# AaltoPML/PPBO

Measured on NVIDIA B200. Metric: ppbo_iteration_ms, lower is better.
Workload: dtype f64

## Files before the change

ppbo_b200/csrc/acq.cu:

```cuda
#include <algorithm>
#include <cmath>
#include <cstdlib>
#include <vector>

#include "../../include/ppbo_b200.h"
#include "common.cuh"
#include "gemm_f64.cuh"
#include "linalg.cuh"
#include "philox.cuh"

namespace ppbo {

extern int g_tuning[16];
int kernel_matvec(int kind, const double* X1, int n1, const double* X2, int n2, int D, const double* ls_h, double sigma_f,
                  const double* alpha, double* mu, double* partial, cudaStream_t st);
int kernel_matrix_raw(int kind, const double* X1, int n1, const double* X2, int n2, int D, const double* ls_h,
                      double sigma_f, double scale, double diag_add, double* out, long long ld, cudaStream_t st);

__global__ void __launch_bounds__(256) pred_diff_kernel(const double* __restrict__ Kc, long long ldk, int PT, int Q, int m,
                                                        const double* __restrict__ arrow, double* __restrict__ Ut,
                                                        long long ldu) {
    const int u = blockIdx.x * blockDim.x + threadIdx.x, p = blockIdx.y;
    if (u >= Q * m) return;
    const int q = u / m, j = u % m;
// ... 153 lines not shown
#pragma unroll
            for (int d = 0; d < RM_MAX_D; ++d)
                if (d < D) gl[d] = fma(c, w[d], gl[d]);
        }
        for (int o = 16; o > 0; o >>= 1) val += __shfl_xor_sync(0xffffffffu, val, o);
        if (lane == 0) red[warp][RM_MAX_D] = val;
#pragma unroll
        for (int d = 0; d < RM_MAX_D; ++d) {
            if (d < D) {
                double v = gl[d];
                for (int o = 16; o > 0; o >>= 1) v += __shfl_xor_sync(0xffffffffu, v, o);
                if (lane == 0) red[warp][d] = v;
            }
        }
        __syncthreads();
        if (tid <= D) {
            const int k = (tid == D) ? RM_MAX_D : tid;
            const double v = amp * ((red[0][k] + red[1][k]) + (red[2][k] + red[3][k]));
            if (tid == D) fval_s = v;
            else gv[tid] = v;
        }
        __syncthreads();
    };
    if (tid < D) x[tid] = fmin(fmax(x0[tid], 0.0), 1.0);
    __syncthreads();
    eval(x, g);
    double f = fval_s;
    double gmax = 0.0;
    for (int d = 0; d < D; ++d) gmax = fmax(gmax, fabs(g[d]));
    double t = 0.05 / fmax(gmax, 1e-12);
    int it = 0;
    for (; it < max_iter; ++it) {
        double pg = 0.0;
        for (int d = 0; d < D; ++d) pg = fmax(pg, fabs(fmin(fmax(x[d] + g[d], 0.0), 1.0) - x[d]));
        if (pg <= gtol) break;
        double ft = f, slope = 0.0;
        int tries = 0;
        for (;; ++tries) {
            __syncthreads();
            if (tid < D) xt[tid] = fmin(fmax(x[tid] + t * g[tid], 0.0), 1.0);
            __syncthreads();
            slope = 0.0;
            for (int d = 0; d < D; ++d) slope = fma(g[d], xt[d] - x[d], slope);
            eval(xt, gt);
            ft = fval_s;
            if (ft >= f + 1e-4 * slope || tries >= 30) break;
            t *= 0.5;
        }
        if (!(ft >= f)) break;
        double ss = 0.0, sy = 0.0;
        for (int d = 0; d < D; ++d) {
            const double sd = xt[d] - x[d], yd = gt[d] - g[d];
            ss = fma(sd, sd, ss);
            sy = fma(sd, yd, sy);
        }
        __syncthreads();
        if (tid < D) { x[tid] = xt[tid]; g[tid] = gt[tid]; }
        __syncthreads();
        f = ft;
        t = (sy < 0.0) ? fmin(fmax(-ss / sy, 1e-8), 1e4) : 2.0 * t;
        if (ss == 0.0) break;
    }
    if (tid < D) xout[(long long)blockIdx.x * D + tid] = x[tid];
    if (tid == 0) {
        fout[blockIdx.x] = f;
        if (iters_out) iters_out[blockIdx.x] = it;
    }
}
__global__ void rff_maximize_select_kernel(const double* __restrict__ xall, const double* __restrict__ fall, int S, int R, int D,
                                           double* __restrict__ xbest, double* __restrict__ fbest) {
    const int s = blockIdx.x * blockDim.x + threadIdx.x;
    if (s >= S) return;
    int br = 0;
    double bf = fall[(long long)s * R];
    for (int r = 1; r < R; ++r) {
        const double v = fall[(long long)s * R + r];
        if (v > bf) { bf = v; br = r; }
    }
    fbest[s] = bf;
    for (int d = 0; d < D; ++d) xbest[(long long)s * D + d] = xall[((long long)s * R + br) * D + d];
}

constexpr int FV_SLICES = 8, FV_COLS = 128;
__global__ void __launch_bounds__(256) rff_fvals_partial_kernel(const double* __restrict__ Phi, long long ld, int F, int N,
                                                                const double* __restrict__ omega, double* __restrict__ part,
                                                                const double* __restrict__ skip) {
    __shared__ double red[FV_COLS];
    if (skip && *skip != 0.0) return;
    const int c = threadIdx.x & (FV_COLS - 1), half = threadIdx.x >> 7;
    const int i = blockIdx.x * FV_COLS + c;
    const int per = (F + FV_SLICES - 1) / FV_SLICES;
    const int f0 = blockIdx.y * per, f1 = min(F, f0 + per);
    double s0 = 0.0, s1 = 0.0;
    if (i < N) {
        int f = f0 + half;
        for (; f + 2 < f1; f += 4) {
            s0 = fma(Phi[(long long)f * ld + i], omega[f], s0);
            s1 = fma(Phi[(long long)(f + 2) * ld + i], omega[f + 2], s1);
        }
        for (; f < f1; f += 2) s0 = fma(Phi[(long long)f * ld + i], omega[f], s0);
    }
    if (half == 1) red[c] = s0 + s1;
    __syncthreads();
    if (half == 0 && i < N) part[(long long)blockIdx.y * N + i] = (s0 + s1) + red[c];
}
__global__ void __launch_bounds__(256) rff_fvals_combine_kernel(const double* __restrict__ part, int N, double* __restrict__ y) {
    const int i = blockIdx.x * blockDim.x + threadIdx.x;
    if (i >= N) return;
    double s = 0.0;
#pragma unroll
    for (int k = 0; k < FV_SLICES; ++k) s += part[(long long)k * N + i];
    y[i] = s;
}
static int launch_rff_fvals(const double* Phi, long long ld, int F, int N, const double* omega, double* part, double* y,
                            cudaStream_t st, const double* skip = nullptr) {
    PPBO_CL rff_fvals_partial_kernel<<<dim3(ceil_div(N, FV_COLS), FV_SLICES), 256, 0, st>>>(Phi, ld, F, N, omega, part, skip);
    PPBO_CL rff_fvals_combine_kernel<<<ceil_div(N, 256), 256, 0, st>>>(part, N, y);
    PPBO_LAUNCH_CHECK();
    return PPBO_OK;
}
__global__ void __launch_bounds__(256) rff_grad_hess_kernel(const double* __restrict__ Phi, long long ld, int F, int Q, int m,
                                                            const double* __restrict__ omega, const double* __restrict__ beta,
                                                            const double* __restrict__ arrow, double* __restrict__ grad,
                                                            double* __restrict__ hdiag, const double* __restrict__ skip) {
    if (skip && *skip != 0.0) return;
    const int f = (blockIdx.x * blockDim.x + threadIdx.x) >> 5, lane = threadIdx.x & 31;
    if (f >= F) return;
    const double* ph = Phi + (long long)f * ld;
    const int N = Q * (m + 1), M = Q * m;
    double g = 0.0, h = 0.0;
    if (grad) for (int i = lane; i < N; i += 32) g = fma(beta[i], ph[i], g);
    if (hdiag)
        for (int u = lane; u < M; u += 32) {
            const int q = u / m, j = u % m;
            const double d = ph[(long long)q * (m + 1) + 1 + j] - ph[(long long)q * (m + 1)];
            h = fma(arrow[u], d * d, h);
        }
    for (int o = 16; o > 0; o >>= 1) {
        g += __shfl_xor_sync(0xffffffffu, g, o);
        h += __shfl_xor_sync(0xffffffffu, h, o);
    }
    if (lane == 0) {
        if (grad) grad[f] = -omega[f] + g;
        if (hdiag) hdiag[f] = -1.0 - h;
    }
}
__global__ void __launch_bounds__(256) rff_grad_kernel(const double* __restrict__ Phi, long long ld, int F, int N,
                                                       const double* __restrict__ omega, const double* __restrict__ beta,
                                                       double* __restrict__ grad, const double* __restrict__ skip) {
    __shared__ double part[8];
    if (skip && *skip != 0.0) return;
    const int warp = threadIdx.x >> 5, lane = threadIdx.x & 31;
    const int f = blockIdx.x * 2 + (warp >> 2), qtr = warp & 3;
    double g0 = 0.0, g1 = 0.0;
    if (f < F) {
        const double* ph = Phi + (long long)f * ld;
        const int per = ((N + 3) / 4 + 31) / 32 * 32, i0 = qtr * per, i1 = min(N, i0 + per);
        int i = i0 + lane;
        for (; i + 32 < i1; i += 64) {
            g0 = fma(beta[i], ph[i], g0);
            g1 = fma(beta[i + 32], ph[i + 32], g1);
        }
        if (i < i1) g0 = fma(beta[i], ph[i], g0);
    }
    double g = g0 + g1;
    for (int o = 16; o > 0; o >>= 1) g += __shfl_xor_sync(0xffffffffu, g, o);
    if (lane == 0) part[warp] = g;
    __syncthreads();
    if (threadIdx.x < 2) {
        const int ff = blockIdx.x * 2 + threadIdx.x;
        if (ff < F) grad[ff] = -omega[ff] + ((part[4 * threadIdx.x] + part[4 * threadIdx.x + 1]) + (part[4 * threadIdx.x + 2] + part[4 * threadIdx.x + 3]));
    }
}
__global__ void __launch_bounds__(256) rff_psi_kernel(const double* __restrict__ Phi, long long ld, int Q, int m,
                                                      const double* __restrict__ arrow, double* __restrict__ PsiT, long long ldp) {
    const int u = blockIdx.x * blockDim.x + threadIdx.x, f = blockIdx.y;
    if (u >= Q * m) return;
    const int q = u / m, j = u % m;
    const double* ph = Phi + (long long)f * ld;
    const double a = arrow[u];
    PsiT[(long long)f * ldp + u] = a > 0.0 ? sqrt(a) * (ph[(long long)q * (m + 1) + 1 + j] - ph[(long long)q * (m + 1)]) : 0.0;
}
__global__ void add_identity_kernel(double* __restrict__ A, long long ld, int n) {
    const int i = blockIdx.x * blockDim.x + threadIdx.x;
    if (i < n) A[(long long)i * ld + i] += 1.0;
}
__global__ void __launch_bounds__(1024) rff_scalars_kernel(const double* __restrict__ omega, const double* __restrict__ x, int F,
                                                           double* __restrict__ scal) {
    __shared__ double red[33];
    __shared__ double mx[2][32];
    double s = 0, m0 = 0, m1 = 0;
    for (int i = threadIdx.x; i < F; i += 1024) {
        s = fma(omega[i], omega[i], s);
        if (x) m0 = fmax(m0, fabs(x[i]));
        m1 = fmax(m1, fabs(omega[i]));
    }
    s = block_sum(s, red);
    for (int o = 16; o > 0; o >>= 1) {
        m0 = fmax(m0, __shfl_xor_sync(0xffffffffu, m0, o));
        m1 = fmax(m1, __shfl_xor_sync(0xffffffffu, m1, o));
    }
    if ((threadIdx.x & 31) == 0) { mx[0][threadIdx.x >> 5] = m0; mx[1][threadIdx.x >> 5] = m1; }
    __syncthreads();
    if (threadIdx.x == 0) {
        for (int w = 1; w < 32; ++w) { m0 = fmax(m0, mx[0][w]); m1 = fmax(m1, mx[1][w]); }
        scal[0] = -0.5 * s; scal[1] = m0; scal[2] = m1;
    }
}
__global__ void axpy_kernel(double* __restrict__ y, const double* __restrict__ x, double a, int n) {
    const int i = blockIdx.x * blockDim.x + threadIdx.x;
    if (i < n) y[i] += a * x[i];
}
__global__ void axpy_out_kernel(double* __restrict__ out, const double* __restrict__ y, const double* __restrict__ x, double a, int n) {
    const int i = blockIdx.x * blockDim.x + threadIdx.x;
    if (i < n) out[i] = y[i] + a * x[i];
}

int launch_lik_terms(const double* f, int Q, int m, double sigma, double* set_lik, double* beta, double* arrow, double* sa,
                     double* bvec, cudaStream_t st);
int launch_sum(const double* x, int n, double* out, cudaStream_t st);
int launch_linesearch_lik(const double* f, const double* df, int Q, int m, double sigma, double* part, cudaStream_t st);
constexpr int LS_STEPS = 8;

__global__ void __launch_bounds__(1024) rff_ls_scalars_kernel(const double* __restrict__ omega, const double* __restrict__ step,
                                                              int F, const double* __restrict__ part, int Q,
                                                              double* __restrict__ scal) {
    __shared__ double red_multi[32 * (3 + LS_STEPS)];
    __shared__ double mx[2][32];
    double m0 = 0, m1 = 0;
    double sums[3 + LS_STEPS];
#pragma unroll
    for (int c = 0; c < 3 + LS_STEPS; ++c) sums[c] = 0.0;
    for (int i = threadIdx.x; i < F; i += 1024) {
        const double o = omega[i], d = step[i];
        sums[0] = fma(o, o, sums[0]);
        sums[1] = fma(o, d, sums[1]);
        sums[2] = fma(d, d, sums[2]);
        m0 = fmax(m0, fabs(d));
        m1 = fmax(m1, fabs(o));
    }
    for (int q = threadIdx.x; q < Q; q += 1024) {
#pragma unroll
        for (int c = 0; c < LS_STEPS; ++c) sums[3 + c] += part[(long long)c * Q + q];
    }
    block_sum_multi<3 + LS_STEPS>(sums, red_multi);
    for (int o = 16; o > 0; o >>= 1) {
        m0 = fmax(m0, __shfl_xor_sync(0xffffffffu, m0, o));
        m1 = fmax(m1, __shfl_xor_sync(0xffffffffu, m1, o));
    }
    if ((threadIdx.x & 31) == 0) { mx[0][threadIdx.x >> 5] = m0; mx[1][threadIdx.x >> 5] = m1; }
    __syncthreads();
    if (threadIdx.x == 0) {
        for (int w = 1; w < 32; ++w) { m0 = fmax(m0, mx[0][w]); m1 = fmax(m1, mx[1][w]); }
        scal[0] = sums[0]; scal[1] = sums[1]; scal[2] = sums[2]; scal[3] = m0; scal[4] = m1;
        for (int c = 0; c < LS_STEPS; ++c) scal[8 + c] = sums[3 + c];
    }
}

__global__ void __launch_bounds__(256) rff_chord_decide_kernel(double* __restrict__ omega, const double* __restrict__ step, int F,
                                                               const double* __restrict__ scal, int m, double* __restrict__ state,
                                                               double* __restrict__ hist, int anderson) {
    __shared__ int accept_s;
    if (state[4] != 0.0) return;
    if (threadIdx.x == 0) {
        const double oo = scal[0], od = scal[1], dd = scal[2], max_step = scal[3], max_om = fmax(scal[4], 1e-300);
        const double S_cur = -0.5 * oo - scal[24] / m;
        const double S1 = -0.5 * (oo + 2.0 * od + dd) - scal[8] / m;
        const int accept = S1 >= S_cur - 1e-13 * fabs(S_cur);
        accept_s = accept;
        state[7] = accept ? 1.0 : 0.0;
        if (!accept) {
            state[4] = 3.0;
        } else {
            const double rel = max_step / max_om, prev = state[1], rel3 = state[3];
            const int n = (int)state[5];
            state[0] = S1;
            state[3] = state[2];
            state[2] = prev;
            state[1] = rel;
            state[5] = n + 1;
            hist[2 * n] = rel;
            hist[2 * n + 1] = S1;
            if (rel <= state[6]) state[4] = 1.0;
            else if (anderson) { if (rel3 < 1e300 && !(rel <= 0.2 * rel3)) state[4] = 2.0; }
            else if (!(rel <= 0.5 * prev)) state[4] = 2.0;
        }
    }
    __syncthreads();
    if (!accept_s) return;
    for (int i = threadIdx.x; i < F; i += blockDim.x) omega[i] += step[i];
}

constexpr int RAA_M = 5;
__global__ void __launch_bounds__(1024) rff_anderson_kernel(double* __restrict__ omega, const double* __restrict__ step, int F,
                                                            const double* __restrict__ state, double* __restrict__ aa,
                                                            double* __restrict__ Hh) {
    __shared__ double gam[RAA_M];
    __shared__ int nh_s;
    if (state[4] != 0.0) return;
    double* dR = Hh;
    double* dG = Hh + (long long)RAA_M * F;
    double* pr = Hh + 2LL * RAA_M * F;
    double* pg = pr + F;
    const bool plain = state[7] == 1.0;
    const double rel = state[1];
    int nh = (int)aa[0], slot = (int)aa[1];
    const double rel_prev = aa[2];
    bool have_prev = aa[3] == 1.0;
    __syncthreads();
    if (!plain || (have_prev && rel > 1.5 * rel_prev)) {
        if (threadIdx.x == 0) { aa[0] = 0.0; aa[1] = 0.0; aa[2] = rel; aa[3] = 0.0; }
        if (!plain) return;
        nh = 0;
        slot = 0;
        have_prev = false;
    }
    if (have_prev) {
        for (int i = threadIdx.x; i < F; i += 1024) {
            dR[(long long)slot * F + i] = step[i] - pr[i];
            dG[(long long)slot * F + i] = omega[i] - pg[i];
        }
        nh = min(nh + 1, RAA_M);
        slot = (slot + 1) % RAA_M;
    }
    for (int i = threadIdx.x; i < F; i += 1024) {
        pr[i] = step[i];
        pg[i] = omega[i];
    }
    __syncthreads();
    constexpr int NPAIR = RAA_M * (RAA_M + 1) / 2;
    __shared__ double red_multi[32 * (NPAIR + RAA_M)];
    double acc[NPAIR + RAA_M];
#pragma unroll
    for (int i = 0; i < NPAIR + RAA_M; ++i) acc[i] = 0.0;
    for (int k = threadIdx.x; k < F; k += 1024) {
        double dv[RAA_M];
#pragma unroll
        for (int i = 0; i < RAA_M; ++i) dv[i] = (i < nh) ? dR[(long long)i * F + k] : 0.0;
        const double rk = step[k];
        int idx = 0;
#pragma unroll
        for (int i = 0; i < RAA_M; ++i) {
#pragma unroll
            for (int j = 0; j <= i; ++j) { acc[idx] = fma(dv[i], dv[j], acc[idx]); ++idx; }
            acc[NPAIR + i] = fma(dv[i], rk, acc[NPAIR + i]);
        }
    }
    block_sum_multi<NPAIR + RAA_M>(acc, red_multi);
    double A[RAA_M][RAA_M], bb[RAA_M];
    {
        int idx = 0;
#pragma unroll
        for (int i = 0; i < RAA_M; ++i) {
#pragma unroll
            for (int j = 0; j <= i; ++j) { A[i][j] = A[j][i] = acc[idx]; ++idx; }
            bb[i] = acc[NPAIR + i];
        }
    }
    if (threadIdx.x == 0) {
        double tr = 0.0;
        for (int i = 0; i < nh; ++i) tr += A[i][i];
        for (int i = 0; i < nh; ++i) A[i][i] += 1e-10 * tr + 1e-300;
        bool ok = true;
        for (int c = 0; c < nh && ok; ++c) {
            int pv = c;
            for (int r2 = c + 1; r2 < nh; ++r2) if (fabs(A[r2][c]) > fabs(A[pv][c])) pv = r2;
            if (A[pv][c] == 0.0) { ok = false; break; }
            for (int k = 0; k < nh; ++k) { const double t = A[c][k]; A[c][k] = A[pv][k]; A[pv][k] = t; }
            { const double t = bb[c]; bb[c] = bb[pv]; bb[pv] = t; }
            for (int r2 = c + 1; r2 < nh; ++r2) {
                const double l = A[r2][c] / A[c][c];
                for (int k = c; k < nh; ++k) A[r2][k] -= l * A[c][k];
                bb[r2] -= l * bb[c];
            }
        }
        for (int i = nh - 1; i >= 0 && ok; --i) {
            double v = bb[i];
            for (int k = i + 1; k < nh; ++k) v -= A[i][k] * gam[k];
            gam[i] = v / A[i][i];
            if (!(fabs(gam[i]) < 1e3)) ok = false;
        }
        nh_s = ok ? nh : 0;
        aa[0] = ok ? nh : 0;
        aa[1] = ok ? slot : 0;
        aa[2] = rel;
        aa[3] = 1.0;
    }
    __syncthreads();
    const int nm = nh_s;
    if (nm == 0) return;
    for (int i = threadIdx.x; i < F; i += 1024) {
        double c = 0.0;
        for (int j = 0; j < nm; ++j) c = fma(gam[j], dG[(long long)j * F + i], c);
        omega[i] -= c;
    }
}

}

using namespace ppbo;

extern "C" long long ppbo_factor_doubles(int n) { return (long long)n * n + potrf_dinv_doubles(n) ; }

extern "C" int ppbo_neg_count(const double* arrow, int M, int* idx_h, int idx_capacity, void* stream) {
    std::vector<double> a((size_t)M);
    if (readback().add(a.data(), arrow, sizeof(double) * M, (cudaStream_t)stream) != cudaSuccess ||
        readback().finish((cudaStream_t)stream) != cudaSuccess) {
        set_error("ppbo_neg_count: copy failed");
        return PPBO_ERR_CUDA;
    }
    int r = 0;
    for (int u = 0; u < M; ++u)
        if (a[u] < 0.0) {
            if (idx_h && r < idx_capacity) idx_h[r] = u;
            ++r;
        }
    return r;
}
extern "C" long long ppbo_neg_corr_doubles(int M, int r) {
    return (long long)((r + 1) / 2) + (long long)r * M + ppbo_factor_doubles(r) + 2;
}
extern "C" int ppbo_neg_corr_build(const double* G, long long ldg, int M, const double* arrow, const double* Lfac, int cap,
                                   const int* idx_h, int r, double* neg_corr, void* stream) {
    if (r <= 0) return PPBO_OK;
    PPBO_REQUIRE(cap >= M && ldg >= M, "capacity / leading dimension below M");
    cudaStream_t st = (cudaStream_t)stream;
    int* idx = reinterpret_cast<int*>(neg_corr);
    double* Ht = neg_corr + (r + 1) / 2;
    double* R = Ht + (long long)r * M;
    double* Rdinv = R + (long long)r * r;
    int* info_d = reinterpret_cast<int*>(neg_corr + ppbo_neg_corr_doubles(M, r) - 1);
    PPBO_CUDA_CHECK(cudaMemcpyAsync(idx, idx_h, sizeof(int) * r, cudaMemcpyHostToDevice, st));
    PPBO_CL neg_rows_kernel<<<dim3(ceil_div(M, 256), r), 256, 0, st>>>(G, ldg, M, arrow, idx, r, Ht, R, r);
    PPBO_LAUNCH_CHECK();
    int rc = trsm_right_lower_t(Lfac, cap, M, Lfac + (long long)cap * cap, Ht, M, r, st);
    if (rc) return rc;
    GemmOperands g{Ht, M, 0, Ht, M, 0, r, r, M};
    StoreEpilogue ep{R, r, 0, 1.0, 1.0, 0, 0, 0};
    if ((rc = launch_gemm_nt(g, ep, 1, st))) return rc;
    if ((rc = potrf_lower(R, r, r, Rdinv, info_d, st))) return rc;
    int info = 0;
    PPBO_CUDA_CHECK(readback().add(&info, info_d, sizeof(int), st));
    PPBO_CUDA_CHECK(readback().finish(st));
    if (info) { set_error("posterior precision is not positive definite (negative-coefficient block, pivot %d)", info); return info; }
    return PPBO_OK;
}

extern "C" long long ppbo_predict_workspace_bytes(int N, int Q, int m, int P, int batch) {
    const long long PT = (long long)P * batch, M = (long long)Q * m;
    return (PT * N + PT * M + PT * M + 64) * 8;
}

extern "C" long long ppbo_predict_mean_workspace_bytes(int kind, int N, int P, int batch) {
    const long long PT = (long long)P * batch;
    if (kind == PPBO_KERNEL_SE || kind == PPBO_KERNEL_RQ) return (PT * ((N + 63) / 64) + 64) * 8;
    return (PT * N + 64) * 8;
}

extern "C" int ppbo_predict(int kind, const double* X, int N, int D, const double* lengthscales_h, double sigma_f,
                            double shrinkage, int Q, int m, const double* alpha, const double* arrow, const double* Lfac, int cap,
                            const double* neg_corr, int n_neg, const double* Xp, int P, int batch, double* mu,
                            double* Sigma_p, void* workspace, long long workspace_bytes, void* stream) {
    PPBO_REQUIRE(N == Q * (m + 1), "N must equal Q (m+1)");
    PPBO_REQUIRE(Sigma_p == nullptr || cap >= Q * m, "factor capacity below Q m");
    PPBO_REQUIRE(P >= 1 && batch >= 1, "empty grid");
    PPBO_REQUIRE(workspace_bytes >= (Sigma_p ? ppbo_predict_workspace_bytes(N, Q, m, P, batch)
                                             : ppbo_predict_mean_workspace_bytes(g_tuning[11] ? PPBO_KERNEL_CAMPHOR : kind, N, P, batch)),
                 "workspace too small");
    cudaStream_t st = (cudaStream_t)stream;
    const int PT = P * batch, M = Q * m;
    double* Kc = (double*)workspace;
    double* Ut = Kc + (long long)PT * N;
    double* Ud = Ut + (long long)PT * M;
    int rc;
    if (!Sigma_p) {
        if (!mu) return PPBO_OK;
        rc = kernel_matvec(kind, Xp, PT, X, N, D, lengthscales_h, sigma_f, alpha, mu, Kc, st);
        if (rc < 0) return rc;
// ... 32 lines not shown
        StoreEpilogue e2{Sigma_p, P, (long long)P * P, 1.0, 1.0, 0, 0, 0};
        if ((rc = launch_gemm_nt(g2, e2, batch, st))) return rc;
    }
    return PPBO_OK;
}

extern "C" int ppbo_mvn_rowmax(const double* Z, long long ldz, long long strideZ, const double* Fac, long long ldf,
                               long long strideF, const double* mu, long long strideMu, int S, int P, int K, int batch,
                               double* fmax, int* arg, void* stream) {
    PPBO_REQUIRE(S >= 0 && P >= 1 && K >= 1 && batch >= 1, "shape");
    GemmOperands g{Z, ldz, strideZ, Fac, ldf, strideF, S, P, K};
    RowMaxEpilogue ep{mu, strideMu, fmax, arg, nullptr, 0, 0};
    return launch_gemm_nt_rowmax(g, ep, batch, (cudaStream_t)stream);
}

extern "C" int ppbo_acq_reduce(const double* fmax, int S, int batch, double mustar, double* out, void* stream) {
    PPBO_REQUIRE(S >= 1 && batch >= 1, "shape");
    PPBO_CL acq_reduce_kernel<<<batch, 1024, 0, (cudaStream_t)stream>>>(fmax, S, mustar, nullptr, out);
    PPBO_LAUNCH_CHECK();
    return PPBO_OK;
}

extern "C" int ppbo_acq_reduce_dev(const double* fmax, int S, int batch, const double* mustar_dev, double* out, void* stream) {
    PPBO_REQUIRE(S >= 1 && batch >= 1 && mustar_dev != nullptr, "shape");
    PPBO_CL acq_reduce_kernel<<<batch, 1024, 0, (cudaStream_t)stream>>>(fmax, S, 0.0, mustar_dev, out);
    PPBO_LAUNCH_CHECK();
    return PPBO_OK;
}

extern "C" int ppbo_vec_max(const double* x, long long n, int accumulate, double* out, void* stream) {
    PPBO_REQUIRE(n >= 0 && out != nullptr, "shape");
    PPBO_CL vec_max_kernel<<<1, 1024, 0, (cudaStream_t)stream>>>(x, n, accumulate, out);
    PPBO_LAUNCH_CHECK();
    return PPBO_OK;
}

extern "C" int ppbo_rff_features(const double* W, const double* b, int F, int D, const double* X, int n, double sigma_f,
                                 double* Phi, long long ld, int feature_major, void* stream) {
    PPBO_REQUIRE(F >= 1 && D >= 1 && n >= 0, "shape");
    if (n == 0) return PPBO_OK;
    const double amp = sqrt(2.0 * sigma_f * sigma_f / F);
    dim3 grid = feature_major ? dim3(ceil_div(n, 256), F) : dim3(ceil_div(F, 256), n);
    PPBO_REQUIRE(grid.y <= 65535, "too many rows for one launch");
    PPBO_CL rff_features_kernel<<<grid, 256, sizeof(double) * D, (cudaStream_t)stream>>>(W, b, F, D, X, n, amp, Phi, ld, feature_major);
    PPBO_LAUNCH_CHECK();
    return PPBO_OK;
}

extern "C" int ppbo_rff_jacobian(const double* W, const double* b, int F, int D, const double* x, double sigma_f, double* J,
                                 void* stream) {
    const double amp = sqrt(2.0 * sigma_f * sigma_f / F);
    PPBO_CL rff_jacobian_kernel<<<ceil_div(F, 128), 128, 0, (cudaStream_t)stream>>>(W, b, F, D, x, amp, J);
    PPBO_LAUNCH_CHECK();
    return PPBO_OK;
}

extern "C" int ppbo_rff_value_grad(const double* W, const double* b, int F, int D, const double* omega, const double* x,
                                   double sigma_f, double* out, void* stream) {
    PPBO_REQUIRE(F >= 1 && D >= 1 && D <= PPBO_MAX_D, "shape");
    const double amp = sqrt(2.0 * sigma_f * sigma_f / F);
    PPBO_CL rff_value_grad_kernel<<<1, 256, 0, (cudaStream_t)stream>>>(W, b, F, D, omega, x, amp, out);
    PPBO_LAUNCH_CHECK();
    return PPBO_OK;
}

extern "C" int ppbo_rff_maximize(const double* W, const double* b, int F, int D, double sigma_f, const double* Omega, long long ldo,
                                 int S, const double* X0, int R, int max_iter, double gtol, double* xbest, double* fbest,
                                 double* work, void* stream) {
    PPBO_REQUIRE(F >= 1 && D >= 1 && D <= RM_MAX_D, "D must be in [1, 32]");
    PPBO_REQUIRE(S >= 0 && R >= 1 && max_iter >= 0 && gtol >= 0 && work != nullptr, "arguments");
    if (S == 0) return PPBO_OK;
    cudaStream_t st = (cudaStream_t)stream;
    const double amp = sqrt(2.0 * sigma_f * sigma_f / F);
    double* xall = work;
    double* fall = work + (long long)S * R * D;
    PPBO_CL rff_maximize_kernel<<<S * R, RM_THREADS, 0, st>>>(W, b, F, D, amp, Omega, ldo, X0, R, max_iter, gtol, xall, fall, nullptr);
    PPBO_CL rff_maximize_select_kernel<<<ceil_div(S, 128), 128, 0, st>>>(xall, fall, S, R, D, xbest, fbest);
    PPBO_LAUNCH_CHECK();
    return PPBO_OK;
}

extern "C" long long ppbo_rff_workspace_bytes(int F, int Q, int m) {
    const long long N = (long long)Q * (m + 1), M = (long long)Q * m;
    return ((3 + FV_SLICES) * N + 2 * M + Q * 9 + 64 + (long long)F * M + ppbo_factor_doubles(F) + 4 * (long long)F + 2 * CHOL_NB +
            blockinv_doubles(F) + (2LL * RAA_M + 2) * F + 8) * 8;
}

struct RffWs {
    double *fvals, *dfv, *fpart, *beta, *arrow, *setlik, *scal, *PsiT, *H, *grad, *step, *trial, *tmp, *binv, *aaH, *aa;
    void carve(double* p, int F, int Q, int m) {
        const long long N = (long long)Q * (m + 1), M = (long long)Q * m;
        fvals = p; p += N;
        dfv = p; p += N;
        fpart = p; p += (long long)FV_SLICES * N;
        beta = p; p += N;
        arrow = p; p += 2 * M;
        setlik = p; p += 9LL * Q;
        scal = p; p += 64;
        PsiT = p; p += (long long)F * M;
        H = p; p += ppbo_factor_doubles(F);
        grad = p; p += F;
        step = p; p += F + CHOL_NB;
        trial = p; p += F;
        tmp = p; p += F;
        aaH = p; p += (2LL * RAA_M + 2) * F;
        aa = p; p += 8;
        binv = p;
    }
};

static int rff_eval(const double* Phi, long long ld, int F, int Q, int m, double sigma, const double* omega, RffWs& ws,
                    double* grad, double* hdiag, bool want_arrow, double* lik_sum_dev, cudaStream_t st, const double* skip = nullptr) {
    const int N = Q * (m + 1);
    launch_rff_fvals(Phi, ld, F, N, omega, ws.fpart, ws.fvals, st, skip);
    launch_lik_terms(ws.fvals, Q, m, sigma, ws.setlik, ws.beta, want_arrow ? ws.arrow : nullptr, nullptr, nullptr, st);
    launch_sum(ws.setlik, Q, lik_sum_dev, st);
    if (grad && !hdiag)
        PPBO_CL rff_grad_kernel<<<ceil_div(F, 2), 256, 0, st>>>(Phi, ld, F, N, omega, ws.beta, grad, skip);
    else if (grad || hdiag)
        PPBO_CL rff_grad_hess_kernel<<<ceil_div(F, 8), 256, 0, st>>>(Phi, ld, F, Q, m, omega, ws.beta, ws.arrow, grad, hdiag, skip);
    PPBO_LAUNCH_CHECK();
    return PPBO_OK;
}

extern "C" int ppbo_rff_objective(const double* Phi_X, long long ld, int F, int Q, int m, double sigma, const double* omega,
                                  double* S_out, double* grad, double* hess_diag, void* workspace, long long workspace_bytes,
                                  void* stream) {
    PPBO_REQUIRE(workspace_bytes >= ppbo_rff_workspace_bytes(F, Q, m), "workspace too small");
    cudaStream_t st = (cudaStream_t)stream;
    RffWs ws;
    ws.carve((double*)workspace, F, Q, m);
    int rc = rff_eval(Phi_X, ld, F, Q, m, sigma, omega, ws, grad, hess_diag, true, ws.scal + 8, st);
    if (rc) return rc;
    if (S_out) {
        PPBO_CL rff_scalars_kernel<<<1, 1024, 0, st>>>(omega, nullptr, F, ws.scal);
        double h[9];
        PPBO_CUDA_CHECK(readback().add(h, ws.scal, sizeof(h), st));
        PPBO_CUDA_CHECK(readback().finish(st));
        *S_out = h[0] - h[8] / m;
    }
    return PPBO_OK;
}

extern "C" long long ppbo_rff_factor_cache_doubles(int F) { return ppbo_factor_doubles(F) + blockinv_doubles(F); }

extern "C" int ppbo_rff_fit(const double* Phi_X, long long ld, int F, int Q, int m, double sigma, const double* omega0,
                            int max_iter, double tol, double* factor_cache, int warm_factor, double* omega_map, double* hess_diag,
                            void* workspace, long long workspace_bytes, double* stats_h, void* stream) {
    PPBO_REQUIRE(workspace_bytes >= ppbo_rff_workspace_bytes(F, Q, m), "workspace too small");
    PPBO_REQUIRE(!warm_factor || (factor_cache != nullptr && omega0 != nullptr), "a warm factor needs the cache and omega0");
    cudaStream_t st = (cudaStream_t)stream;
    const int M = Q * m;
    RffWs ws;
    ws.carve((double*)workspace, F, Q, m);
    if (factor_cache) {
        ws.H = factor_cache;
        ws.binv = factor_cache + ppbo_factor_doubles(F);
    }
    double* Hdinv = ws.H + (long long)F * F;
    int* info_d = reinterpret_cast<int*>(ws.scal + 32);
    PPBO_CUDA_CHECK(cudaMemsetAsync(info_d, 0, sizeof(int), st));
    if (omega0) PPBO_CUDA_CHECK(cudaMemcpyAsync(omega_map, omega0, sizeof(double) * F, cudaMemcpyDeviceToDevice, st));
    else PPBO_CUDA_CHECK(cudaMemsetAsync(omega_map, 0, sizeof(double) * F, st));
    int rc, it = 0, info = 0, n_factor = 0, n_chord = 0;
    double h[32], S_cur = NAN, last_rel = INFINITY;
    const int N = Q * (m + 1);
    double* part = ws.setlik + Q;
    const double CHORD_REL = 0.25;
    const bool trace = getenv("PPBO_TRACE") != nullptr;
    bool refactor = !warm_factor, binv_valid = warm_factor == 2;
    constexpr int RFF_BATCH_MAX = 8;
    double* state_d = ws.scal + 40;
    double* hist_d = ws.scal + 48;
    double prev_rel_h = INFINITY, rel3_h = INFINITY;
    bool first_batch = true;
    const bool anderson = !(getenv("PPBO_RFF_ANDERSON") && atoi(getenv("PPBO_RFF_ANDERSON")) == 0);
    PPBO_CUDA_CHECK(cudaMemsetAsync(ws.aa, 0, sizeof(double) * 8, st));
    for (it = 0; it < max_iter; ++it) {
        if (!refactor) {
            if (!binv_valid) {
                if ((rc = blockinv_build(ws.H, F, F, Hdinv, ws.binv, st))) return rc;
                binv_valid = true;
            }
            double rho = (std::isfinite(prev_rel_h) && last_rel < prev_rel_h) ? last_rel / prev_rel_h : 0.2;
            rho = std::fmin(std::fmax(rho, 0.02), anderson ? 0.7 : 0.5);
            int kb = !std::isfinite(last_rel) ? 3 : (last_rel > tol) ? (int)std::ceil(std::log(tol / last_rel) / std::log(rho)) : 1;
            if (first_batch) kb = std::min(kb, 3);
            kb = std::max(1, std::min(kb, std::min(RFF_BATCH_MAX, max_iter - it)));
            first_batch = false;
            double state_h[8] = {S_cur, last_rel, prev_rel_h, rel3_h, 0.0, 0.0, tol, 0.0}, hist_h[2 * RFF_BATCH_MAX];
            PPBO_CUDA_CHECK(cudaMemcpyAsync(state_d, state_h, sizeof(state_h), cudaMemcpyHostToDevice, st));
            const double* skip = state_d + 4;
            for (int i = 0; i < kb; ++i) {
                if ((rc = rff_eval(Phi_X, ld, F, Q, m, sigma, omega_map, ws, ws.grad, nullptr, false, ws.scal + 24, st, skip))) return rc;
                PPBO_CUDA_CHECK(cudaMemcpyAsync(ws.step, ws.grad, sizeof(double) * F, cudaMemcpyDeviceToDevice, st));
                if ((rc = potrs_vec_blockinv(ws.H, F, F, ws.binv, ws.step, st, skip))) return rc;
                launch_rff_fvals(Phi_X, ld, F, N, ws.step, ws.fpart, ws.dfv, st, skip);
                if ((rc = launch_linesearch_lik(ws.fvals, ws.dfv, Q, m, sigma, part, st))) return rc;
                PPBO_CL rff_ls_scalars_kernel<<<1, 1024, 0, st>>>(omega_map, ws.step, F, part, Q, ws.scal);
                PPBO_CL rff_chord_decide_kernel<<<1, 256, 0, st>>>(omega_map, ws.step, F, ws.scal, m, state_d, hist_d, anderson ? 1 : 0);
                if (anderson) PPBO_CL rff_anderson_kernel<<<1, 1024, 0, st>>>(omega_map, ws.step, F, state_d, ws.aa, ws.aaH);
            }
            PPBO_LAUNCH_CHECK();
            PPBO_CUDA_CHECK(readback().add(state_h, state_d, sizeof(state_h), st));
            PPBO_CUDA_CHECK(readback().add(hist_h, hist_d, sizeof(double) * 2 * kb, st));
            PPBO_CUDA_CHECK(readback().finish(st));
            const int taken = (int)state_h[5], stop = (int)state_h[4];
            if (trace)
                for (int i = 0; i < taken; ++i)
                    fprintf(stderr, "[ppbo_rff_fit] it %d chord  step 1 rel %.3e S %.12g (batch of %d)\n", it + i, hist_h[2 * i], hist_h[2 * i + 1], kb);
            n_chord += taken;
            if (taken > 0) {
                last_rel = state_h[1];
                prev_rel_h = state_h[2];
                rel3_h = state_h[3];
            }
            S_cur = (stop == 1 || !anderson) ? (taken > 0 ? state_h[0] : S_cur) : NAN;
            it += taken;
            if (stop == 1) break;
            if (stop == 2 || stop == 3) refactor = true;
            --it;
            continue;
        }
        if ((rc = rff_eval(Phi_X, ld, F, Q, m, sigma, omega_map, ws, ws.grad, nullptr, true, ws.scal + 24, st))) return rc;
        PPBO_CL rff_psi_kernel<<<dim3(ceil_div(M, 256), F), 256, 0, st>>>(Phi_X, ld, Q, m, ws.arrow, ws.PsiT, M);
        {
            GemmOperands g{ws.PsiT, M, 0, ws.PsiT, M, 0, F, F, M};
            StoreEpilogue ep{ws.H, F, 0, 1.0, 0.0, 2, 0, 0};
            if ((rc = launch_gemm_nt(g, ep, 1, st))) return rc;
        }
        PPBO_CL add_identity_kernel<<<ceil_div(F, 256), 256, 0, st>>>(ws.H, F, F);
        if ((rc = potrf_lower(ws.H, F, F, Hdinv, info_d, st))) return rc;
        ++n_factor;
        binv_valid = false;
        PPBO_CUDA_CHECK(cudaMemsetAsync(ws.aa, 0, sizeof(double) * 8, st));
        rel3_h = INFINITY;
        PPBO_CUDA_CHECK(cudaMemcpyAsync(ws.step, ws.grad, sizeof(double) * F, cudaMemcpyDeviceToDevice, st));
        if ((rc = potrs_vec(ws.H, F, F, Hdinv, ws.step, st))) return rc;
        launch_rff_fvals(Phi_X, ld, F, N, ws.step, ws.fpart, ws.dfv, st);
        if ((rc = launch_linesearch_lik(ws.fvals, ws.dfv, Q, m, sigma, part, st))) return rc;
        PPBO_CL rff_ls_scalars_kernel<<<1, 1024, 0, st>>>(omega_map, ws.step, F, part, Q, ws.scal);
        PPBO_LAUNCH_CHECK();
        PPBO_CUDA_CHECK(readback().add(h, ws.scal, sizeof(double) * 32, st));
        PPBO_CUDA_CHECK(readback().add(&info, info_d, sizeof(int), st));
        PPBO_CUDA_CHECK(readback().finish(st));
        if (info) { set_error("weight-space Hessian not positive definite (pivot %d)", info); return info; }
        const double oo = h[0], od = h[1], dd = h[2], max_step = h[3], max_om = fmax(h[4], 1e-300);
        if (std::isnan(S_cur)) S_cur = -0.5 * oo - h[24] / m;
        int c;
        double s = 1.0, S_new = S_cur;
        for (c = 0; c < LS_STEPS; ++c) {
            s = std::ldexp(1.0, -c);
            const double S_try = -0.5 * (oo + 2.0 * s * od + s * s * dd) - h[8 + c] / m;
            if (S_try >= S_cur - 1e-13 * fabs(S_cur)) { S_new = S_try; break; }
        }
        if (c == LS_STEPS) { s = std::ldexp(1.0, -(LS_STEPS - 1)); S_new = NAN; }
        PPBO_CL axpy_kernel<<<ceil_div(F, 256), 256, 0, st>>>(omega_map, ws.step, s, F);
        PPBO_LAUNCH_CHECK();
        S_cur = S_new;
        prev_rel_h = last_rel;
        last_rel = s * max_step / max_om;
        if (trace) fprintf(stderr, "[ppbo_rff_fit] it %d newton step %.3g rel %.3e S %.12g\n", it, s, last_rel, S_cur);
        if (c == 0 && last_rel <= tol) { ++it; break; }
        refactor = !(c == 0 && last_rel <= CHORD_REL);
    }
    if (std::isnan(S_cur)) {
        if ((rc = rff_eval(Phi_X, ld, F, Q, m, sigma, omega_map, ws, nullptr, nullptr, false, ws.scal + 24, st))) return rc;
        PPBO_CL rff_scalars_kernel<<<1, 1024, 0, st>>>(omega_map, nullptr, F, ws.scal);
        PPBO_CUDA_CHECK(readback().add(h, ws.scal, sizeof(double) * 32, st));
        PPBO_CUDA_CHECK(readback().finish(st));
        S_cur = h[0] - h[24] / m;
    }
    if (hess_diag) {
        if ((rc = rff_eval(Phi_X, ld, F, Q, m, sigma, omega_map, ws, nullptr, hess_diag, true, ws.scal + 24, st))) return rc;
    }
    PPBO_CUDA_CHECK(readback().finish(st));
    if (stats_h) {
        stats_h[0] = it; stats_h[1] = last_rel; stats_h[2] = S_cur; stats_h[3] = n_factor + 0.001 * n_chord;
        stats_h[4] = (binv_valid && factor_cache) ? 1.0 : 0.0;
    }
    return PPBO_OK;
}

extern "C" int ppbo_rff_refactor(const double* Phi_X, long long ld, int F, int Q, int m, double sigma, const double* omega,
                                 double* factor_cache, void* workspace, long long workspace_bytes, void* stream) {
    PPBO_REQUIRE(workspace_bytes >= ppbo_rff_workspace_bytes(F, Q, m) && factor_cache != nullptr, "workspace / cache");
    cudaStream_t st = (cudaStream_t)stream;
    const int M = Q * m;
    RffWs ws;
    ws.carve((double*)workspace, F, Q, m);
    ws.H = factor_cache;
    ws.binv = factor_cache + ppbo_factor_doubles(F);
    double* Hdinv = ws.H + (long long)F * F;
    int* info_d = reinterpret_cast<int*>(ws.scal + 32);
    int rc;
    if ((rc = rff_eval(Phi_X, ld, F, Q, m, sigma, omega, ws, nullptr, nullptr, true, ws.scal + 24, st))) return rc;
    PPBO_CL rff_psi_kernel<<<dim3(ceil_div(M, 256), F), 256, 0, st>>>(Phi_X, ld, Q, m, ws.arrow, ws.PsiT, M);
    GemmOperands g{ws.PsiT, M, 0, ws.PsiT, M, 0, F, F, M};
    StoreEpilogue ep{ws.H, F, 0, 1.0, 0.0, 2, 0, 0};
    if ((rc = launch_gemm_nt(g, ep, 1, st))) return rc;
    PPBO_CL add_identity_kernel<<<ceil_div(F, 256), 256, 0, st>>>(ws.H, F, F);
    PPBO_LAUNCH_CHECK();
    if ((rc = potrf_lower(ws.H, F, F, Hdinv, info_d, st))) return rc;
    return blockinv_build(ws.H, F, F, Hdinv, ws.binv, st);
}

extern "C" int ppbo_rff_eval_argmax(const double* Omega, long long ldo, int S, int F, const double* PhiT_grid, long long ldp,
                                    long long stridePhi, int P, int batch, double* fmax, int* arg, double* Fs_full,
                                    void* stream) {
    PPBO_REQUIRE(S >= 0 && F >= 1 && P >= 1 && batch >= 1, "shape");
    GemmOperands g{Omega, ldo, 0, PhiT_grid, ldp, stridePhi, S, P, F};
    RowMaxEpilogue ep{nullptr, 0, fmax, arg, Fs_full, P, (long long)S * P};
    return launch_gemm_nt_rowmax(g, ep, batch, (cudaStream_t)stream);
}

namespace ppbo {

__global__ void __launch_bounds__(256) normal_fill_kernel(unsigned long long seed, uint32_t stream, long long offset,
                                                          double* __restrict__ out, long long n) {
    const long long first = offset >> 1, last = (offset + n - 1) >> 1;
    for (long long c = first + (long long)blockIdx.x * blockDim.x + threadIdx.x; c <= last;
         c += (long long)gridDim.x * blockDim.x) {
        double z0, z1;
        philox_normal2(seed, (unsigned long long)c, stream, z0, z1);
        const long long e0 = 2 * c - offset, e1 = e0 + 1;
        if (e0 >= 0 && e0 < n) out[e0] = z0;
        if (e1 >= 0 && e1 < n) out[e1] = z1;
    }
}

__global__ void __launch_bounds__(256) sample_omega_kernel(const double* __restrict__ omega_map,
                                                           const double* __restrict__ hess_diag,
                                                           const double* __restrict__ Z, long long ldz,
                                                           unsigned long long seed, uint32_t stream, long long sample0, int S,
                                                           int F, double* __restrict__ Omega, long long ldo) {
    const int s = blockIdx.y;
    const int fp = blockIdx.x * blockDim.x + threadIdx.x;
    const int f0 = 2 * fp;
    if (f0 >= F) return;
    double z0, z1 = 0.0;
    if (Z) {
        z0 = Z[(long long)s * ldz + f0];
        if (f0 + 1 < F) z1 = Z[(long long)s * ldz + f0 + 1];
    } else {
        const long long e = (sample0 + s) * (long long)F + f0;
        if ((e & 1) == 0) {
            philox_normal2(seed, (unsigned long long)(e >> 1), stream, z0, z1);
        } else {
            double a, b;
            philox_normal2(seed, (unsigned long long)(e >> 1), stream, a, b);
            z0 = b;
            philox_normal2(seed, (unsigned long long)((e + 1) >> 1), stream, a, b);
            z1 = a;
        }
    }
    double* o = Omega + (long long)s * ldo;
    o[f0] = omega_map[f0] + z0 * rsqrt(-hess_diag[f0]);
    if (f0 + 1 < F) o[f0 + 1] = omega_map[f0 + 1] + z1 * rsqrt(-hess_diag[f0 + 1]);
}

}

extern "C" int ppbo_normal_fill(unsigned long long seed, unsigned int stream_id, long long offset, double* out, long long n,
                                void* stream) {
    PPBO_REQUIRE(n >= 0 && offset >= 0, "shape");
    if (n == 0) return PPBO_OK;
    const long long counters = ((offset + n - 1) >> 1) - (offset >> 1) + 1;
    const int blocks = (int)std::min<long long>(ceil_div_ll(counters, 256), PPBO_SM_COUNT * 16);
    PPBO_CL normal_fill_kernel<<<blocks, 256, 0, (cudaStream_t)stream>>>(seed, stream_id, offset, out, n);
    PPBO_LAUNCH_CHECK();
    return PPBO_OK;
}

extern "C" int ppbo_rff_sample_omega(const double* omega_map, const double* hess_diag, const double* Z, long long ldz,
                                     unsigned long long seed, unsigned int stream_id, long long sample0, int S, int F,
                                     double* Omega, long long ldo, void* stream) {
    PPBO_REQUIRE(S >= 0 && F >= 1 && ldo >= F, "shape");
// ... 13 lines not shown
```

Measured before the change: 16.22.

## Fuse RFF fvals combine and chord tail kernels, skip first Hessian build

Result: faster. 15.58 (median of 6 runs) (-4.0%).

```diff
diff --git a/ppbo_b200/csrc/acq.cu b/ppbo_b200/csrc/acq.cu
--- a/ppbo_b200/csrc/acq.cu
+++ b/ppbo_b200/csrc/acq.cu
@@ -259,10 +259,11 @@
 }
 
 constexpr int FV_SLICES = 8, FV_COLS = 128;
-__global__ void __launch_bounds__(256) rff_fvals_partial_kernel(const double* __restrict__ Phi, long long ld, int F, int N,
-                                                                const double* __restrict__ omega, double* __restrict__ part,
-                                                                const double* __restrict__ skip) {
+__global__ void __launch_bounds__(256) rff_fvals_kernel(const double* __restrict__ Phi, long long ld, int F, int N,
+                                                        const double* __restrict__ omega, double* part, double* __restrict__ y,
+                                                        unsigned* __restrict__ count, const double* __restrict__ skip) {
     __shared__ double red[FV_COLS];
+    __shared__ bool last;
     if (skip && *skip != 0.0) return;
     const int c = threadIdx.x & (FV_COLS - 1), half = threadIdx.x >> 7;
     const int i = blockIdx.x * FV_COLS + c;
@@ -280,19 +281,24 @@
     if (half == 1) red[c] = s0 + s1;
     __syncthreads();
     if (half == 0 && i < N) part[(long long)blockIdx.y * N + i] = (s0 + s1) + red[c];
-}
-__global__ void __launch_bounds__(256) rff_fvals_combine_kernel(const double* __restrict__ part, int N, double* __restrict__ y) {
-    const int i = blockIdx.x * blockDim.x + threadIdx.x;
-    if (i >= N) return;
-    double s = 0.0;
+    __threadfence();
+    __syncthreads();
+    if (threadIdx.x == 0) last = atomicAdd(count + blockIdx.x, 1u) == FV_SLICES - 1;
+    __syncthreads();
+    if (!last) return;
+    __threadfence();
+    if (half == 0 && i < N) {
+        double s = 0.0;
 #pragma unroll
-    for (int k = 0; k < FV_SLICES; ++k) s += part[(long long)k * N + i];
-    y[i] = s;
-}
+        for (int k = 0; k < FV_SLICES; ++k) s += __ldcg(part + (long long)k * N + i);
+        y[i] = s;
+    }
+    if (threadIdx.x == 0) count[blockIdx.x] = 0u;
+}
+static int fvals_count_words(int N) { return ceil_div(N, FV_COLS); }
 static int launch_rff_fvals(const double* Phi, long long ld, int F, int N, const double* omega, double* part, double* y,
-                            cudaStream_t st, const double* skip = nullptr) {
-    PPBO_CL rff_fvals_partial_kernel<<<dim3(ceil_div(N, FV_COLS), FV_SLICES), 256, 0, st>>>(Phi, ld, F, N, omega, part, skip);
-    PPBO_CL rff_fvals_combine_kernel<<<ceil_div(N, 256), 256, 0, st>>>(part, N, y);
+                            unsigned* count, cudaStream_t st, const double* skip = nullptr) {
+    PPBO_CL rff_fvals_kernel<<<dim3(ceil_div(N, FV_COLS), FV_SLICES), 256, 0, st>>>(Phi, ld, F, N, omega, part, y, count, skip);
     PPBO_LAUNCH_CHECK();
     return PPBO_OK;
 }
@@ -399,9 +405,8 @@
 int launch_linesearch_lik(const double* f, const double* df, int Q, int m, double sigma, double* part, cudaStream_t st);
 constexpr int LS_STEPS = 8;
 
-__global__ void __launch_bounds__(1024) rff_ls_scalars_kernel(const double* __restrict__ omega, const double* __restrict__ step,
-                                                              int F, const double* __restrict__ part, int Q,
-                                                              double* __restrict__ scal) {
+__device__ __forceinline__ void rff_ls_scalars(const double* omega, const double* __restrict__ step, int F,
+                                               const double* __restrict__ part, int Q, double* scal) {
     __shared__ double red_multi[32 * (3 + LS_STEPS)];
     __shared__ double mx[2][32];
     double m0 = 0, m1 = 0;
@@ -433,12 +438,15 @@
         for (int c = 0; c < LS_STEPS; ++c) scal[8 + c] = sums[3 + c];
     }
 }
-
-__global__ void __launch_bounds__(256) rff_chord_decide_kernel(double* __restrict__ omega, const double* __restrict__ step, int F,
-                                                               const double* __restrict__ scal, int m, double* __restrict__ state,
-                                                               double* __restrict__ hist, int anderson) {
+__global__ void __launch_bounds__(1024) rff_ls_scalars_kernel(const double* __restrict__ omega, const double* __restrict__ step,
+                                                              int F, const double* __restrict__ part, int Q,
+                                                              double* __restrict__ scal) {
+    rff_ls_scalars(omega, step, F, part, Q, scal);
+}
+
+__device__ __forceinline__ bool rff_chord_decide(double* omega, const double* __restrict__ step, int F, const double* scal, int m,
+                                                 double* state, double* hist, int anderson) {
     __shared__ int accept_s;
-    if (state[4] != 0.0) return;
     if (threadIdx.x == 0) {
         const double oo = scal[0], od = scal[1], dd = scal[2], max_step = scal[3], max_om = fmax(scal[4], 1e-300);
         const double S_cur = -0.5 * oo - scal[24] / m;
@@ -464,14 +472,14 @@
         }
     }
     __syncthreads();
-    if (!accept_s) return;
+    if (!accept_s) return false;
     for (int i = threadIdx.x; i < F; i += blockDim.x) omega[i] += step[i];
+    return true;
 }
 
 constexpr int RAA_M = 5;
-__global__ void __launch_bounds__(1024) rff_anderson_kernel(double* __restrict__ omega, const double* __restrict__ step, int F,
-                                                            const double* __restrict__ state, double* __restrict__ aa,
-                                                            double* __restrict__ Hh) {
+__device__ __forceinline__ void rff_anderson(double* omega, const double* __restrict__ step, int F, const double* state, double* aa,
+                                             double* Hh) {
     __shared__ double gam[RAA_M];
     __shared__ int nh_s;
     if (state[4] != 0.0) return;
@@ -571,6 +579,23 @@
         for (int j = 0; j < nm; ++j) c = fma(gam[j], dG[(long long)j * F + i], c);
         omega[i] -= c;
     }
+}
+
+__global__ void __launch_bounds__(1024) rff_chord_tail_kernel(double* omega, const double* __restrict__ step, int F,
+                                                              const double* __restrict__ setlik, const double* __restrict__ part,
+                                                              int Q, int m, double* scal, double* state, double* hist, int anderson,
+                                                              double* aa, double* Hh) {
+    __shared__ double red[33];
+    if (state[4] != 0.0) return;
+    double s = 0.0;
+    for (int i = threadIdx.x; i < Q; i += 1024) s += setlik[i];
+    s = block_sum(s, red);
+    if (threadIdx.x == 0) scal[24] = s;
+    rff_ls_scalars(omega, step, F, part, Q, scal);
+    __syncthreads();
+    if (!rff_chord_decide(omega, step, F, scal, m, state, hist, anderson) || !anderson) return;
+    __syncthreads();
+    rff_anderson(omega, step, F, state, aa, Hh);
 }
 
 }
@@ -769,12 +794,14 @@
 
 extern "C" long long ppbo_rff_workspace_bytes(int F, int Q, int m) {
     const long long N = (long long)Q * (m + 1), M = (long long)Q * m;
-    return ((3 + FV_SLICES) * N + 2 * M + Q * 9 + 64 + (long long)F * M + ppbo_factor_doubles(F) + 4 * (long long)F + 2 * CHOL_NB +
-            blockinv_doubles(F) + (2LL * RAA_M + 2) * F + 8) * 8;
+    return ((3 + FV_SLICES) * N + 2 * M + Q * 9 + 64 + (long long)F * M + ppbo_factor_doubles(F) + 3 * (long long)F + 2 * CHOL_NB +
+            blockinv_doubles(F) + (2LL * RAA_M + 2) * F + 8 + (fvals_count_words((int)N) + 1) / 2) * 8;
 }
 
 struct RffWs {
-    double *fvals, *dfv, *fpart, *beta, *arrow, *setlik, *scal, *PsiT, *H, *grad, *step, *trial, *tmp, *binv, *aaH, *aa;
+    double *fvals, *dfv, *fpart, *beta, *arrow, *setlik, *scal, *PsiT, *H, *step, *trial, *tmp, *binv, *aaH, *aa;
+    unsigned* fv_count;
+    int nfv_count;
     void carve(double* p, int F, int Q, int m) {
         const long long N = (long long)Q * (m + 1), M = (long long)Q * m;
         fvals = p; p += N;
@@ -786,22 +813,24 @@
         scal = p; p += 64;
         PsiT = p; p += (long long)F * M;
         H = p; p += ppbo_factor_doubles(F);
-        grad = p; p += F;
         step = p; p += F + CHOL_NB;
         trial = p; p += F;
         tmp = p; p += F;
         aaH = p; p += (2LL * RAA_M + 2) * F;
         aa = p; p += 8;
-        binv = p;
-    }
+        binv = p; p += blockinv_doubles(F);
+        fv_count = reinterpret_cast<unsigned*>(p);
+        nfv_count = fvals_count_words((int)N);
+    }
+    cudaError_t zero_counters(cudaStream_t st) { return cudaMemsetAsync(fv_count, 0, sizeof(unsigned) * nfv_count, st); }
 };
 
 static int rff_eval(const double* Phi, long long ld, int F, int Q, int m, double sigma, const double* omega, RffWs& ws,
                     double* grad, double* hdiag, bool want_arrow, double* lik_sum_dev, cudaStream_t st, const double* skip = nullptr) {
     const int N = Q * (m + 1);
-    launch_rff_fvals(Phi, ld, F, N, omega, ws.fpart, ws.fvals, st, skip);
+    launch_rff_fvals(Phi, ld, F, N, omega, ws.fpart, ws.fvals, ws.fv_count, st, skip);
     launch_lik_terms(ws.fvals, Q, m, sigma, ws.setlik, ws.beta, want_arrow ? ws.arrow : nullptr, nullptr, nullptr, st);
-    launch_sum(ws.setlik, Q, lik_sum_dev, st);
+    if (lik_sum_dev) launch_sum(ws.setlik, Q, lik_sum_dev, st);
     if (grad && !hdiag)
         PPBO_CL rff_grad_kernel<<<ceil_div(F, 2), 256, 0, st>>>(Phi, ld, F, N, omega, ws.beta, grad, skip);
     else if (grad || hdiag)
@@ -817,6 +846,7 @@
     cudaStream_t st = (cudaStream_t)stream;
     RffWs ws;
     ws.carve((double*)workspace, F, Q, m);
+    PPBO_CUDA_CHECK(ws.zero_counters(st));
     int rc = rff_eval(Phi_X, ld, F, Q, m, sigma, omega, ws, grad, hess_diag, true, ws.scal + 8, st);
     if (rc) return rc;
     if (S_out) {
@@ -847,6 +877,7 @@
     double* Hdinv = ws.H + (long long)F * F;
     int* info_d = reinterpret_cast<int*>(ws.scal + 32);
     PPBO_CUDA_CHECK(cudaMemsetAsync(info_d, 0, sizeof(int), st));
+    PPBO_CUDA_CHECK(ws.zero_counters(st));
     if (omega0) PPBO_CUDA_CHECK(cudaMemcpyAsync(omega_map, omega0, sizeof(double) * F, cudaMemcpyDeviceToDevice, st));
     else PPBO_CUDA_CHECK(cudaMemsetAsync(omega_map, 0, sizeof(double) * F, st));
     int rc, it = 0, info = 0, n_factor = 0, n_chord = 0;
@@ -879,14 +910,12 @@
             PPBO_CUDA_CHECK(cudaMemcpyAsync(state_d, state_h, sizeof(state_h), cudaMemcpyHostToDevice, st));
             const double* skip = state_d + 4;
             for (int i = 0; i < kb; ++i) {
-                if ((rc = rff_eval(Phi_X, ld, F, Q, m, sigma, omega_map, ws, ws.grad, nullptr, false, ws.scal + 24, st, skip))) return rc;
-                PPBO_CUDA_CHECK(cudaMemcpyAsync(ws.step, ws.grad, sizeof(double) * F, cudaMemcpyDeviceToDevice, st));
+                if ((rc = rff_eval(Phi_X, ld, F, Q, m, sigma, omega_map, ws, ws.step, nullptr, false, nullptr, st, skip))) return rc;
                 if ((rc = potrs_vec_blockinv(ws.H, F, F, ws.binv, ws.step, st, skip))) return rc;
-                launch_rff_fvals(Phi_X, ld, F, N, ws.step, ws.fpart, ws.dfv, st, skip);
+                launch_rff_fvals(Phi_X, ld, F, N, ws.step, ws.fpart, ws.dfv, ws.fv_count, st, skip);
                 if ((rc = launch_linesearch_lik(ws.fvals, ws.dfv, Q, m, sigma, part, st))) return rc;
-                PPBO_CL rff_ls_scalars_kernel<<<1, 1024, 0, st>>>(omega_map, ws.step, F, part, Q, ws.scal);
-                PPBO_CL rff_chord_decide_kernel<<<1, 256, 0, st>>>(omega_map, ws.step, F, ws.scal, m, state_d, hist_d, anderson ? 1 : 0);
-                if (anderson) PPBO_CL rff_anderson_kernel<<<1, 1024, 0, st>>>(omega_map, ws.step, F, state_d, ws.aa, ws.aaH);
+                PPBO_CL rff_chord_tail_kernel<<<1, 1024, 0, st>>>(omega_map, ws.step, F, ws.setlik, part, Q, m, ws.scal, state_d, hist_d,
+                                                                 anderson ? 1 : 0, ws.aa, ws.aaH);
             }
             PPBO_LAUNCH_CHECK();
             PPBO_CUDA_CHECK(readback().add(state_h, state_d, sizeof(state_h), st));
@@ -909,22 +938,24 @@
             --it;
             continue;
         }
-        if ((rc = rff_eval(Phi_X, ld, F, Q, m, sigma, omega_map, ws, ws.grad, nullptr, true, ws.scal + 24, st))) return rc;
-        PPBO_CL rff_psi_kernel<<<dim3(ceil_div(M, 256), F), 256, 0, st>>>(Phi_X, ld, Q, m, ws.arrow, ws.PsiT, M);
-        {
-            GemmOperands g{ws.PsiT, M, 0, ws.PsiT, M, 0, F, F, M};
-            StoreEpilogue ep{ws.H, F, 0, 1.0, 0.0, 2, 0, 0};
-            if ((rc = launch_gemm_nt(g, ep, 1, st))) return rc;
-        }
-        PPBO_CL add_identity_kernel<<<ceil_div(F, 256), 256, 0, st>>>(ws.H, F, F);
-        if ((rc = potrf_lower(ws.H, F, F, Hdinv, info_d, st))) return rc;
-        ++n_factor;
-        binv_valid = false;
-        PPBO_CUDA_CHECK(cudaMemsetAsync(ws.aa, 0, sizeof(double) * 8, st));
-        rel3_h = INFINITY;
-        PPBO_CUDA_CHECK(cudaMemcpyAsync(ws.step, ws.grad, sizeof(double) * F, cudaMemcpyDeviceToDevice, st));
-        if ((rc = potrs_vec(ws.H, F, F, Hdinv, ws.step, st))) return rc;
-        launch_rff_fvals(Phi_X, ld, F, N, ws.step, ws.fpart, ws.dfv, st);
+        const bool identity_step = it == 0 && omega0 == nullptr;
+        if ((rc = rff_eval(Phi_X, ld, F, Q, m, sigma, omega_map, ws, ws.step, nullptr, !identity_step, ws.scal + 24, st))) return rc;
+        if (!identity_step) {
+            PPBO_CL rff_psi_kernel<<<dim3(ceil_div(M, 256), F), 256, 0, st>>>(Phi_X, ld, Q, m, ws.arrow, ws.PsiT, M);
+            {
+                GemmOperands g{ws.PsiT, M, 0, ws.PsiT, M, 0, F, F, M};
+                StoreEpilogue ep{ws.H, F, 0, 1.0, 0.0, 2, 0, 0};
+                if ((rc = launch_gemm_nt(g, ep, 1, st))) return rc;
+            }
+            PPBO_CL add_identity_kernel<<<ceil_div(F, 256), 256, 0, st>>>(ws.H, F, F);
+            if ((rc = potrf_lower(ws.H, F, F, Hdinv, info_d, st))) return rc;
+            ++n_factor;
+            binv_valid = false;
+            PPBO_CUDA_CHECK(cudaMemsetAsync(ws.aa, 0, sizeof(double) * 8, st));
+            rel3_h = INFINITY;
+            if ((rc = potrs_vec(ws.H, F, F, Hdinv, ws.step, st))) return rc;
+        }
+        launch_rff_fvals(Phi_X, ld, F, N, ws.step, ws.fpart, ws.dfv, ws.fv_count, st);
         if ((rc = launch_linesearch_lik(ws.fvals, ws.dfv, Q, m, sigma, part, st))) return rc;
         PPBO_CL rff_ls_scalars_kernel<<<1, 1024, 0, st>>>(omega_map, ws.step, F, part, Q, ws.scal);
         PPBO_LAUNCH_CHECK();
@@ -949,7 +980,7 @@
         last_rel = s * max_step / max_om;
         if (trace) fprintf(stderr, "[ppbo_rff_fit] it %d newton step %.3g rel %.3e S %.12g\n", it, s, last_rel, S_cur);
         if (c == 0 && last_rel <= tol) { ++it; break; }
-        refactor = !(c == 0 && last_rel <= CHORD_REL);
+        refactor = identity_step || !(c == 0 && last_rel <= CHORD_REL);
     }
     if (std::isnan(S_cur)) {
         if ((rc = rff_eval(Phi_X, ld, F, Q, m, sigma, omega_map, ws, nullptr, nullptr, false, ws.scal + 24, st))) return rc;
@@ -980,6 +1011,7 @@
     ws.binv = factor_cache + ppbo_factor_doubles(F);
     double* Hdinv = ws.H + (long long)F * F;
     int* info_d = reinterpret_cast<int*>(ws.scal + 32);
+    PPBO_CUDA_CHECK(ws.zero_counters(st));
     int rc;
     if ((rc = rff_eval(Phi_X, ld, F, Q, m, sigma, omega, ws, nullptr, nullptr, true, ws.scal + 24, st))) return rc;
     PPBO_CL rff_psi_kernel<<<dim3(ceil_div(M, 256), F), 256, 0, st>>>(Phi_X, ld, Q, m, ws.arrow, ws.PsiT, M);
```
